# Chthi/Ofighters

Measured on AMD Instinct MI355X. Metric: arena-steps/sec (env.step+obs+policy fwd) at 4096 arenas, 1/2/4/8 MI355X, higher is better.
Workload: dtype f32; 1 GPU; 4096 arenas x 8 ships per GPU, random-bot actions + step + 2D obs rasterise (u8 maps) + bi-head policy forward for 8 ship(s)/arena, trunk shared per arena (BASELINE configs[3]); arenas_per_gpu=4096, ships=8, laser_cap=512, episode_ticks=200, parallelism=arena-sharded x1, RCCL all-reduce of episodic scores only, laser_overflow=0, last_episode_score_sum=70993, last_episode_arenas=4096

## Files before the change

### include/ofx.h

```cpp
#ifndef OFX_H
#define OFX_H

#include <stddef.h>
#include <stdint.h>

#ifdef __cplusplus
extern "C" {
#endif

#define OFX_VERSION 1

enum {
  OFX_OK = 0,
  OFX_ERR_INVALID = -1,
  OFX_ERR_NO_DEVICE = -2,
  OFX_ERR_HIP = -3,
  OFX_ERR_STATE = -4,
  OFX_ERR_OVERFLOW = -5
};

typedef struct ofx_config {
  int32_t n_arenas;
  int32_t n_ships;
  int32_t laser_cap;
// ... 103 lines not shown
int ofx_map_desc(ofx_handle *h, int map_type, int which, ofx_tensor_desc *out);

int ofx_overflow_count(ofx_handle *h, int64_t *count_host);

int ofx_episode_scores(ofx_handle *h, int64_t *sums);
int ofx_episode_scores_grouped(ofx_handle *h, const int32_t *group, int32_t n_groups, int64_t *sums);
int ofx_scores_allreduce(ofx_handle *h, void *nccl_comm, int64_t *sums);

int ofx_scratch_feed(ofx_handle *h, const int32_t *layers_host, int32_t n_layers,
                     const double *weights, const double *biases, const double *x,
                     int32_t batch, double *y, int32_t *argmax);
int ofx_scratch_feed_obs(ofx_handle *h, const int32_t *layers_host, int32_t n_layers,
                         const double *weights, const double *biases, double *y,
                         int32_t *argmax);

typedef struct ofx_policy_desc {
  int32_t n_floats;
  int32_t offset[64];
  int32_t count[64];
  int32_t n_tensors;
} ofx_policy_desc;
int ofx_policy_layout(const ofx_handle *h, ofx_policy_desc *desc_host);
int ofx_policy_forward(ofx_handle *h, const float *weights, const uint8_t *ship_mask,
                       float *act_values, int32_t *iaction, int32_t *ipointer,
                       float *heatmap);
int ofx_policy_pin_weights(ofx_handle *h, const float *weights);
#define OFX_OPT_TRUNK_PLAIN 1
#define OFX_OPT_FRAMES_REF  2
#define OFX_OPT_TRUNK_FUSE  4
#define OFX_OPT_BILINEAR_LEGACY 3
#define OFX_OPT_POLICY_BF16 5
#define OFX_OPT_FIT_PLAIN 6
#define OFX_OPT_TRUNK_SPARSE 7
int ofx_policy_trunk_stats(ofx_handle *h, int64_t *counts_host);
int ofx_set_option(ofx_handle *h, int32_t option, int32_t value);
int ofx_policy_explore(ofx_handle *h, double epsilon, uint64_t seed, uint32_t tick, int32_t collecting,
                       const uint8_t *ship_mask, int32_t *iaction, int32_t *ipointer);
int ofx_policy_epsilon_ladder(ofx_handle *h, const double *expo_host);
int ofx_policy_epsilon_ladder_host(ofx_handle *h, double *dst_host);
int ofx_policy_act(ofx_handle *h, const float *weights, const uint8_t *ship_mask, double epsilon, uint64_t seed,
                   uint32_t tick, int32_t collecting, float *q_sa, float *p_sp, float *v_act, float *v_ptr);
int ofx_policy_actions(ofx_handle *h, const int32_t *iaction, const int32_t *ipointer,
                       const uint8_t *ship_mask, ofx_action *actions);

typedef struct ofx_transition {
  int32_t tick_prev, tick_next;
  int32_t frame_prev, frame_next;
  int32_t ship;
  int32_t iaction, px, py;
  int32_t reward;
  int32_t done;
  float head_prev[8], head_next[8];
} ofx_transition;
int ofx_replay_create(ofx_handle *h, int32_t capacity, int32_t frames);
int ofx_replay_destroy(ofx_handle *h);
int ofx_replay_capture(ofx_handle *h, uint32_t tick, const uint8_t *ship_mask, const int32_t *iaction,
                       const int32_t *ipointer);
int ofx_agents_first_done(ofx_handle *h, const uint8_t *ship_mask, uint8_t *seen, int32_t *count_host);
int ofx_replay_count(ofx_handle *h, int32_t *count_host, int64_t *appended_host);
int ofx_replay_rows_host(ofx_handle *h, int32_t arena, ofx_transition *rows_host, int32_t *n_host);
int ofx_replay_frame_host(ofx_handle *h, int32_t arena, int32_t tick, void *ship_bits_host, void *laser_bits_host);
int ofx_replay_sample(ofx_handle *h, uint64_t seed, uint32_t draw, int32_t batch, int32_t *slot, int32_t *n_sampled);
int ofx_replay_gather(ofx_handle *h, const int32_t *slot, int32_t batch, ofx_transition *rows, void *bits_prev,
                      void *bits_next);
int ofx_replay_gather_valid(ofx_handle *h, const int32_t *slot, const int32_t *n_sampled, int32_t batch, int32_t first,
                            int32_t max_rows, ofx_transition *rows, void *bits_prev, void *bits_next,
// ... 89 lines not shown
```

### ofighters_amd/_native.py

```python
import ctypes as C
import os

_HERE = os.path.dirname(os.path.abspath(__file__))
LIB_PATH = os.path.join(_HERE, "libofx.so")

OFX_OK = 0
OFX_ERR_INVALID = -1
OFX_ERR_NO_DEVICE = -2
OFX_ERR_HIP = -3
OFX_ERR_STATE = -4
OFX_ERR_OVERFLOW = -5

BOT_IDLE, BOT_RANDOM, BOT_TURRET, BOT_RUNNER, BOT_THRUST, BOT_SHOOT = range(6)
BEHAVIOURS = {None: BOT_IDLE, "idle": BOT_IDLE, "random": BOT_RANDOM, "turret": BOT_TURRET,
              "runner": BOT_RUNNER, "thrust": BOT_THRUST, "shoot": BOT_SHOOT}

(F_SHIP_X, F_SHIP_Y, F_SHIP_PX, F_SHIP_PY, F_SHIP_ALIVE, F_REWARD, F_SCORE, F_N_LASERS, F_LASER_X, F_LASER_Y,
 F_LASER_OWNER, F_LASER_DEAD, F_KILLER, F_TIME, F_LAST_SCORES, F_HULL, F_LASER_DX, F_LASER_DY,
 F_OBS_REWARD) = range(19)

MAP_U8, MAP_F32, MAP_F64, MAP_BITS = range(4)
OPT_TRUNK_PLAIN, OPT_FRAMES_REF, OPT_BILINEAR_LEGACY, OPT_TRUNK_FUSE, OPT_POLICY_BF16, OPT_FIT_PLAIN, OPT_TRUNK_SPARSE = 1, 2, 3, 4, 5, 6, 7


class OfxError(Exception):
    def __init__(self, code, msg):
        super().__init__(msg)
        self.code = code


class OfxConfig(C.Structure):
    _fields_ = [(n, C.c_int32) for n in (
        "n_arenas", "n_ships", "laser_cap", "width", "height", "ship_radius", "laser_radius",
        "ship_speed", "laser_speed", "reward_death", "reward_kill", "reward_aim",
        "reward_trajectory", "episode_ticks", "device", "arena_base")]


class OfxAction(C.Structure):
    _fields_ = [("px", C.c_int32), ("py", C.c_int32), ("shoot", C.c_uint8), ("thrust", C.c_uint8),
                ("valid", C.c_uint8), ("_pad", C.c_uint8)]


class OfxTransition(C.Structure):
    _fields_ = [("tick_prev", C.c_int32), ("tick_next", C.c_int32), ("frame_prev", C.c_int32),
                ("frame_next", C.c_int32), ("ship", C.c_int32), ("iaction", C.c_int32),
                ("px", C.c_int32), ("py", C.c_int32), ("reward", C.c_int32), ("done", C.c_int32),
                ("head_prev", C.c_float * 8), ("head_next", C.c_float * 8)]


class OfxTensorDesc(C.Structure):
    _fields_ = [("data", C.c_void_p), ("dtype", C.c_int32), ("itemsize", C.c_int32), ("ndim", C.c_int32),
                ("device", C.c_int32), ("shape", C.c_int64 * 4), ("stride", C.c_int64 * 4)]


DT_U8, DT_I16, DT_I32, DT_I64, DT_F32, DT_F64 = range(6)
# ... 139 lines not shown
```

### ofighters_amd/csrc/ofx_head.hip

```cpp
#include "ofx_head.h"
#include "ofx_lowp.h"
#include "ofx_diag.h"
#include <stdlib.h>


typedef float f32x4 __attribute__((ext_vector_type(4)));
typedef float f32x2 __attribute__((ext_vector_type(2)));
#define HD_PS 400
constexpr int HC4_ZERO = 800;
constexpr int HC4_COL = 816, HC4_CPITCH = 416;
constexpr int HC4_STRIDE = HC4_COL + 2 * HC4_CPITCH + 16;
__device__ __forceinline__ int hc4_at(int ln, int t) { return ln < 2 ? ln * 400 + t : HC4_COL + (ln - 2) * HC4_CPITCH + t; }
__device__ __forceinline__ int hc4_pad(int k) { return k < 16 ? HC4_ZERO + k : k < 32 ? HC4_COL + 400 + k - 16 : HC4_COL + HC4_CPITCH + 400 + k - 32; }

__device__ __forceinline__ void hc4_zero_block(const HeadParams2 &p, int tid, int threads) {
  if (blockIdx.x == 0)
    for (int e = tid; e < HC4_STRIDE; e += threads) p.c4[(size_t)p.S * HC4_STRIDE + e] = 0.f;
}

__device__ __forceinline__ float hd_max_raw(float x, float floor) {
  float pinf;
  asm("s_mov_b32 %0, 0x7f800000" : "=s"(pinf));
  return __builtin_amdgcn_fmed3f(x, floor, pinf);
}

__device__ __forceinline__ unsigned hd_ordered_f32(float v) {
  const unsigned u = __float_as_uint(v);
  return (u & 0x80000000u) ? ~u : (u | 0x80000000u);
}

__global__ __launch_bounds__(1024) void k_head_compact(int S, const uint8_t *mask, int32_t *live) {
  __shared__ int cnt[1024];
  const int t = threadIdx.x, per = (S + 1023) / 1024, lo = min(t * per, S), hi = min(lo + per, S);
  int c = 0;
  for (int s = lo; s < hi; s++) c += mask[s] != 0;
  cnt[t] = c;
  __syncthreads();
  for (int d = 1; d < 1024; d <<= 1) {
    const int v = t >= d ? cnt[t - d] : 0;
    __syncthreads();
    cnt[t] += v;
    __syncthreads();
  }
  int o = cnt[t] - c;
  for (int s = lo; s < hi; s++)
    if (mask[s]) live[1 + o++] = s;
  if (t == 1023) live[0] = cnt[1023];
}

__device__ __forceinline__ int hd_ship(const HeadParams2 &p, int i) {
  if (p.live) return i < p.live[0] ? p.live[1 + i] : -1;
  return i < p.S ? i : -1;
}


__device__ __forceinline__ void hf_taps(int u, int n, int &ka, int &kb, float &w, int legacy) {
  const int k = u >> 1;
  if (legacy) { ka = k; kb = k + 1; w = (u & 1) ? 0.5f : 0.f; }
  else if (u & 1) { ka = k; kb = k + 1; w = 0.25f; } else { ka = k - 1; kb = k; w = 0.75f; }
  ka = min(max(ka, 0), n - 1);
  kb = min(max(kb, 0), n - 1);
}
__device__ __forceinline__ float hf_up(const float *L, int stride, int n, int u, int legacy) {
  int ka, kb; float w;
  hf_taps(u, n, ka, kb, w, legacy);
  const float a = L[ka * stride], b = L[kb * stride];
  return a + (b - a) * w;
}

constexpr int HF_THREADS = 512;
constexpr int HF_L1 = 0;
constexpr int HF_U1R = HF_L1 + 5000;
constexpr int HF_U1C = HF_U1R + 6 * 2 * 102;
constexpr int HF_A_END = HF_U1C + 6 * 2 * 102;
constexpr int HF_U2R = 0;
constexpr int HF_U2C = HF_U2R + 4 * 4 * 202;
static_assert(HF_U2C + 4 * 4 * 202 <= HF_A_END, "region A");
constexpr int HF_B2R = HF_A_END;
constexpr int HF_B2C = HF_B2R + 1600;
constexpr int HF_U3L = HF_B2C + 1600;
constexpr int HF_TOTAL = HF_U3L + 6400;

__global__ __launch_bounds__(HF_THREADS) void k_head_frames_ref(HeadParams2 p) {
  __shared__ __align__(16) float sm[HF_TOTAL];
  const int tid = threadIdx.x;
  const int s = hd_ship(p, (int)blockIdx.x);
  hc4_zero_block(p, tid, HF_THREADS);
  if (s < 0) return;
  float *l1 = sm + HF_L1, *U1r = sm + HF_U1R, *U1c = sm + HF_U1C, *U2r = sm + HF_U2R, *U2c = sm + HF_U2C;
  float *u2rb = sm + HF_B2R, *u2cb = sm + HF_B2C, *u3l = sm + HF_U3L;

  for (int e = tid; e < 5000; e += HF_THREADS) l1[e] = p.up1[(size_t)s * 5000 + e];
  __syncthreads();

  for (int e = tid; e < 2 * 6 * 2 * 102; e += HF_THREADS) {
// ... 101 lines not shown
  __syncthreads();
  for (int e = tid; e < 4 * 200 * 9; e += HF_THREADS) {
    const int tp = e % 9, cell = e / 9;
    float acc = 0.f;
    for (int ci = 0; ci < 8; ci++) acc = fmaf(p.w4raw[tp * 8 + ci], u3l[cell * 8 + ci], acc);
    p.vfr[(size_t)s * 7200 + e] = acc;
  }

  for (int e = tid; e < 4 * 400; e += HF_THREADS) {
    const int ln = e / 400, t = e - ln * 400, isc = ln >> 1, side = ln & 1;
    float acc = 0.f;
    if (!isc || (t > 0 && t < 399)) {
      const int d0 = side ? 2 : 0;
#pragma unroll
      for (int d1 = 0; d1 < 3; d1++)
#pragma unroll
        for (int ci = 0; ci < 8; ci++) {
          const int tap = isc ? d1 * 3 + d0 : d0 * 3 + d1;
          acc += p.w4raw[tap * 8 + ci] * hf_up(u3l + ln * 1600 + ci, 8, 200, t + d1 - 1, p.legacy);
        }
      if (!isc && (t == 0 || t == 399)) {
        const int cl = t ? 3 : 2, dx = t ? 2 : 0;
        for (int dy = 0; dy < 3; dy++) {
          if (dy == d0) continue;
          const int yy = (side ? 399 : 0) + dy - 1;
          if (yy < 0 || yy > 399) continue;
          for (int ci = 0; ci < 8; ci++) acc += p.w4raw[(dy * 3 + dx) * 8 + ci] * hf_up(u3l + cl * 1600 + ci, 8, 200, yy, p.legacy);
        }
      }
    }
    p.c4[(size_t)s * HC4_STRIDE + hc4_at(ln, t)] = acc;
  }
  if (tid < 64) p.c4[(size_t)s * HC4_STRIDE + hc4_pad(tid)] = 0.f;
}

constexpr int HG_THREADS = 256;
constexpr int HG_L1 = 0;
constexpr int HG_U3 = 0;
constexpr int HG_RB = 6400;
constexpr int HG_CB = HG_RB + 4 * 102 * 4;
constexpr int HG_TOTAL = HG_CB + 4 * 102 * 4;
static_assert(2 * 52 * 52 <= 6400, "l1p fits under u3l");

template <int CIN, int COUT, class G>
__device__ __forceinline__ float hg_corner(G get, int n, int yc, int xc, const float *w, float bias, int co, int legacy) {
  float acc = bias;
  for (int dy = 0; dy < 3; dy++) {
    const int uy = yc + dy - 1;
    if (uy < 0 || uy >= 2 * n) continue;
    int ya, yb; float wy;
    hf_taps(uy, n, ya, yb, wy, legacy);
    for (int dx = 0; dx < 3; dx++) {
      const int ux = xc + dx - 1;
      if (ux < 0 || ux >= 2 * n) continue;
      int xa, xb; float wx;
      hf_taps(ux, n, xa, xb, wx, legacy);
      for (int ci = 0; ci < CIN; ci++) {
        const float a = get(ya, xa, ci), b = get(ya, xb, ci), d = get(yb, xa, ci), g = get(yb, xb, ci);
        const float top = a + (b - a) * wx, bot = d + (g - d) * wx;
        acc += w[((dy * 3 + dx) * CIN + ci) * COUT + co] * (top + (bot - top) * wy);
      }
    }
  }
  return fmaxf(acc, 0.f);
}

__global__ __launch_bounds__(HG_THREADS) void k_head_frames(HeadParams2 p) {
  __shared__ __align__(16) float sm[HG_TOTAL];
  __shared__ float efr_s[192], w4s[72];
  const int s = hd_ship(p, (int)((blockIdx.x & ~7u) | ((blockIdx.x + (blockIdx.x >> 3)) & 7u)));
  const int tid = threadIdx.x, lane = tid & 63;
  hc4_zero_block(p, tid, HG_THREADS);
  if (s < 0) return;
  const int wv = __builtin_amdgcn_readfirstlane(tid >> 6);
  const int n16 = lane & 15, kq = lane >> 4;
  float *l1p = sm + HG_L1, *u2rb = sm + HG_RB, *u2cb = sm + HG_CB, *u3l = sm + HG_U3;

  {
    constexpr int NB = 6 * 52 + 46 * 6, NE = 2 * NB, PER = (NE + HG_THREADS - 1) / HG_THREADS;
    float v[PER];
    int at[PER];
#pragma unroll
    for (int u = 0; u < PER; u++) {
      const int e = min(u * HG_THREADS + tid, NE - 1);
      const int ci = e / NB, k = e - ci * NB;
      int r, c;
      if (k < 6 * 52) { const int rr = k / 52; r = rr < 3 ? rr : rr + 46; c = k - rr * 52; }
      else { const int k2 = k - 6 * 52, cc = k2 % 6; r = 3 + k2 / 6; c = cc < 3 ? cc : cc + 46; }
      at[u] = (ci * 52 + r) * 52 + c;
      v[u] = p.up1[(size_t)s * 5000 + (ci * 50 + min(max(r - 1, 0), 49)) * 50 + min(max(c - 1, 0), 49)];
    }
#pragma unroll
    for (int u = 0; u < PER; u++)
      if (u * HG_THREADS + tid < NE) l1p[at[u]] = v[u];
  }
  if (tid < 192) efr_s[tid] = p.efr[tid];
  if (tid < 72) w4s[tid] = p.w4raw[tid];
// ... 668 lines not shown

int ofx_head_compact(ofx_handle *h, int S, const uint8_t *mask, int32_t *live) {
  hipLaunchKernelGGL(k_head_compact, dim3(1), dim3(1024), 0, h->stream, S, mask, live);
  OFX_HIP(hipGetLastError());
  return OFX_OK;
}

size_t ofx_head_frame_bytes(size_t S, size_t *u2fr, size_t *vfr, size_t *c4) {
  *u2fr = 4 * S * 1600;
  *vfr = 4 * S * 7200;
  *c4 = 4 * (S + 1) * HC4_STRIDE;
  return *u2fr + *vfr + *c4;
}

int ofx_launch_head(ofx_handle *h, const HeadParams2 &p0) {
  HeadParams2 p = p0;
#if OFX_HEAD_HOOKS
  { const char *e = getenv("OFX_HEAD_ABLATE"); p.ablate = e ? atoi(e) : 0; }
  static unsigned long long *dbg = nullptr;
  static int dbg_calls = 0;
  const unsigned dbg_blocks = (unsigned)(((p.S + 7) / 8) * 16);
  p.dbg = nullptr;
  if (getenv("OFX_HEAD_STAMPS")) {
    if (!dbg) (void)hipMalloc(&dbg, (size_t)dbg_blocks * 6 * (HS_NB + 4) * 8);
    if (++dbg_calls == 20) p.dbg = dbg;
  }
#endif
  if (p.mask) {
    if (!p.live) { ofx_set_error("ofx_launch_head: a mask needs the live-list scratch"); return OFX_ERR_STATE; }
    if (!p.live_ready) hipLaunchKernelGGL(k_head_compact, dim3(1), dim3(1024), 0, h->stream, p.S, p.mask, p.live);
  } else {
    p.live = nullptr;
  }
  if (p.frames_ref) hipLaunchKernelGGL(k_head_frames_ref, dim3((unsigned)p.S), dim3(HF_THREADS), 0, h->stream, p);
  else hipLaunchKernelGGL(k_head_frames, dim3((unsigned)((p.S + 7) & ~7)), dim3(HG_THREADS), 0, h->stream, p);
  OFX_HIP(hipGetLastError());
  const unsigned blocks = (unsigned)(((p.S + 7) / 8) * 16);
  int rc;
  if (p.event_base >= 0 && (rc = ofx_event_record(h, p.event_base))) return rc;
  const bool extra = p.heat || p.ptr_probe;
#define HS_LAUNCH(E, L) hipLaunchKernelGGL((k_head_stream<E, L>), dim3(blocks), dim3(HS_THREADS), 0, h->stream, p)
  if (p.bf16 == 1) { if (extra) HS_LAUNCH(true, 1); else HS_LAUNCH(false, 1); }
  else if (p.bf16 == 2) { if (extra) HS_LAUNCH(true, 2); else HS_LAUNCH(false, 2); }
  else { if (extra) HS_LAUNCH(true, 0); else HS_LAUNCH(false, 0); }
#undef HS_LAUNCH
  OFX_HIP(hipGetLastError());
  if (p.event_base >= 0 && (rc = ofx_event_record(h, p.event_base + 1))) return rc;
#if OFX_HEAD_HOOKS
  if (p.dbg) {
    (void)hipStreamSynchronize(h->stream);
    unsigned long long *hst = (unsigned long long *)malloc((size_t)blocks * 6 * (HS_NB + 4) * 8);
    (void)hipMemcpy(hst, p.dbg, (size_t)blocks * 6 * (HS_NB + 4) * 8, hipMemcpyDeviceToHost);
    double sum[2][6] = {{0}};
    for (unsigned b = 0; b < blocks; b++)
      for (int w = 0; w < HS_NB + 4; w++)
        for (int i = 0; i < 6; i++) sum[w >= HS_NB][i] += (double)hst[((size_t)b * (HS_NB + 4) + w) * 6 + i] / (w >= HS_NB ? 4.0 : (double)HS_NB);
    for (int r = 0; r < 2; r++) {
      fprintf(stderr, "head stamps %s (cycles per wave and sub-step):", r ? "C" : "B");
      for (int i = 0; i < 6; i++) fprintf(stderr, " %.0f", sum[r][i] / ((double)blocks * HS_NS));
      fprintf(stderr, "\n");
    }
    free(hst);
  }
#endif
  return OFX_OK;
}
```

### ofighters_amd/csrc/ofx_internal.h

```cpp
#pragma once
#include <hip/hip_runtime.h>
#include <stdint.h>
#include <stdio.h>

#include "../../include/ofx.h"

#define OFX_WAVE 64
#define OFX_ARENAS_PER_BLOCK 4

void ofx_set_error(const char *fmt, ...);

#define OFX_HIP(call)                                                                  \
  do {                                                                                 \
    hipError_t _e = (call);                                                            \
    if (_e != hipSuccess) {                                                            \
      ofx_set_error("%s failed: %s (%s:%d)", #call, hipGetErrorString(_e), __FILE__,   \
                    __LINE__);                                                         \
      return OFX_ERR_HIP;                                                              \
    }                                                                                  \
  } while (0)

struct ofx_state {
  int32_t *ship_x, *ship_y, *ship_px, *ship_py, *hull;
  int32_t *reward, *score, *obs_reward, *last_score;
// ... 13 lines not shown
  hipStream_t stream;
  bool own_stream;
  bool spawned;
  ofx_state st;
  double hit_thresh;
  void *maps[5][2];
  int32_t *bot_behaviours;
  void *scratch;
  size_t scratch_bytes;
  hipEvent_t ev0, ev1;
  bool events;
  hipEvent_t *ring;
  int ring_n;
  int prof_base;
  ofx_replay *replay;
  void *aux;
  size_t aux_bytes;
  void *fitws;
  size_t fitws_bytes;
  void *fitws2;
  size_t fitws2_bytes;
  void *applyws;
  size_t applyws_bytes;
  int32_t *counter;
  int32_t *res_iaction;
  int32_t *res_ipointer;
  float *prep;
  float *prep_tmp;
  const float *prep_pinned;
  int opt_trunk_fuse;
  int n_cus;
  bool opt_trunk_plain, opt_frames_ref, opt_bilinear_legacy;
  int opt_policy_lowp;
  bool opt_fit_plain;
  bool opt_trunk_dense, opt_trunk_count;
  unsigned long long *trunk_stat;
  float *act_vals;
  bool act_called;
  double *eps_expo;
};
#define OFX_RING_MAX 65536

int ofx_launch_step(ofx_handle *h, const ofx_action *actions);
int ofx_launch_raster(ofx_handle *h, int map_type, void *ship_map, void *laser_map);
int ofx_ensure_buffer(ofx_handle *h, void **buf, size_t *have, size_t bytes);
int ofx_ensure_scratch(ofx_handle *h, size_t bytes);
enum { OFX_COUNTER_PADS, OFX_COUNTER_FIRST_DONE };
int ofx_counter(ofx_handle *h, int slot, int32_t **counter);
int ofx_policy_results(ofx_handle *h, int32_t **iaction, int32_t **ipointer);
int ofx_policy_act_values(ofx_handle *h, const float **q_sa, const float **p_sp, const float **v_act, const float **v_ptr);
void ofx_replay_free(ofx_handle *h);
int ofx_replay_episode_reset(ofx_handle *h, const uint8_t *arena_mask);
int ofx_launch_gemm(ofx_handle *h, const float *A, int lda, const float *B, int ldb, const float *bias, float *C, int ldc,
                    int M, int N, int K, int relu, const int32_t *live = nullptr);
int ofx_policy_weights_updated(ofx_handle *h, const float *weights);
int ofx_policy_predict_obs(ofx_handle *h, const float *weights, int32_t n_obs, const void *bits, const float *vec8,
                           float *act_values, float *heatmap, float *ptr_max);

#define OFX_MAP_BITS_LSB 4

__host__ __device__ inline void ofx_philox4x32_10(uint32_t c0, uint32_t c1, uint32_t c2, uint32_t c3,
                                                  uint32_t k0, uint32_t k1, uint32_t out[4]) {
#pragma unroll
  for (int r = 0; r < 10; r++) {
    uint64_t p0 = (uint64_t)0xD2511F53u * c0, p1 = (uint64_t)0xCD9E8D57u * c2;
    uint32_t n0 = (uint32_t)(p1 >> 32) ^ c1 ^ k0, n1 = (uint32_t)p1;
// ... 14 lines not shown
```

### ofighters_amd/csrc/ofx_policy.hip

```cpp
#include <string.h>

#include "ofx_internal.h"
#include "ofx_blob.h"
#include "ofx_trunk.h"
#include "ofx_head.h"

typedef float f32x16 __attribute__((ext_vector_type(16)));


extern "C" int ofx_policy_layout(const ofx_handle *h, ofx_policy_desc *desc) {
  (void)h;
  if (!desc) { ofx_set_error("ofx_policy_layout: null desc"); return OFX_ERR_INVALID; }
  memset(desc, 0, sizeof(*desc));
  desc->n_tensors = policy_layout(desc->offset, desc->count);
  desc->n_floats = desc->offset[desc->n_tensors];
  return OFX_OK;
}

struct PrepLayout {
  int tw[4], tb[4];
  int uw[3], ub[3];
  int w3mf;
  int w2mf;
  int w2fr;
  int w3fr;
  int w4eff_c;
  int w4raw;
  int efr;
  int b4;
  int zero16;
  int wbm[3];
  int lut1;
  int total;
};

static PrepLayout prep_layout() {
  PrepLayout L;
  int off = 0;
// ... 440 lines not shown
  pp.legacy = h->opt_bilinear_legacy;
  pp.phase = 0;
  hipLaunchKernelGGL(k_policy_prepare, dim3(32), dim3(256), 0, h->stream, pp);
  pp.phase = 1;
  hipLaunchKernelGGL(k_policy_prepare, dim3(4), dim3(256), 0, h->stream, pp);
  OFX_HIP(hipGetLastError());
  return OFX_OK;
}

extern "C" int ofx_policy_pin_weights(ofx_handle *h, const float *weights) {
  if (!h) { ofx_set_error("ofx_policy_pin_weights: null handle"); return OFX_ERR_INVALID; }
  OFX_HIP(hipSetDevice(h->cfg.device));
  h->prep_pinned = nullptr;
  if (!weights) return OFX_OK;
  int rc = policy_prepare(h, weights, &h->prep);
  if (rc) return rc;
  h->prep_pinned = weights;
  return OFX_OK;
}

int ofx_policy_weights_updated(ofx_handle *h, const float *weights) {
  if (h->prep_pinned && h->prep_pinned == weights) return policy_prepare(h, weights, &h->prep);
  return OFX_OK;
}

extern "C" int ofx_set_option(ofx_handle *h, int32_t option, int32_t value) {
  if (!h) { ofx_set_error("ofx_set_option: null handle"); return OFX_ERR_INVALID; }
  switch (option) {
    case OFX_OPT_TRUNK_PLAIN: h->opt_trunk_plain = value != 0; return OFX_OK;
    case OFX_OPT_TRUNK_FUSE:
      if (value < 0 || value > 2) { ofx_set_error("ofx_set_option: OFX_OPT_TRUNK_FUSE takes 0 (auto), 1 (always), 2 (never)"); return OFX_ERR_INVALID; }
      h->opt_trunk_fuse = value; return OFX_OK;
    case OFX_OPT_FRAMES_REF: h->opt_frames_ref = value != 0; return OFX_OK;
    case OFX_OPT_TRUNK_SPARSE:
      if (value && !h->trunk_stat) {
        OFX_HIP(hipSetDevice(h->cfg.device));
        OFX_HIP(hipMalloc((void **)&h->trunk_stat, 4 * sizeof(unsigned long long)));
        OFX_HIP(hipMemsetAsync(h->trunk_stat, 0, 4 * sizeof(unsigned long long), h->stream));
      }
      h->opt_trunk_dense = value == 0; h->opt_trunk_count = value != 0; return OFX_OK;
    case OFX_OPT_FIT_PLAIN: h->opt_fit_plain = value != 0; return OFX_OK;
    case OFX_OPT_POLICY_BF16:
      if (value < 0 || value > 2) { ofx_set_error("ofx_set_option: OFX_OPT_POLICY_BF16 takes 0 (fp32), 1 (bf16 operands), 2 (fp16 operands)"); return OFX_ERR_INVALID; }
      h->opt_policy_lowp = value; return OFX_OK;
    case OFX_OPT_BILINEAR_LEGACY:
      if (h->opt_bilinear_legacy == (value != 0)) return OFX_OK;
      h->opt_bilinear_legacy = value != 0;
      OFX_HIP(hipSetDevice(h->cfg.device));
      return h->prep_pinned ? policy_prepare(h, h->prep_pinned, &h->prep) : OFX_OK;
    default: ofx_set_error("ofx_set_option: unknown option %d", option); return OFX_ERR_INVALID;
  }
}

struct ForwardArgs {
  const float *weights;
  int N, M;
  const unsigned *bits[2];
  size_t bits_stride;
  const float *vec8;
  const uint8_t *ship_mask;
  float *act_values, *heatmap, *ptr_max, *ptr_probe;
  int32_t *iaction, *ipointer;
  const int32_t *probe;
};

static int policy_forward_impl(ofx_handle *h, const ForwardArgs &a) {
// ... 15 lines not shown
  memset(&tp, 0, sizeof(tp));
  tp.bits[0] = a.bits[0]; tp.bits[1] = a.bits[1]; tp.bits_stride = a.bits_stride; tp.images = N;
  for (int i = 0; i < 4; i++) { tp.tw[i] = prep + L.tw[i]; tp.tb[i] = prep + L.tb[i]; }
  for (int i = 0; i < 3; i++) tp.wbm[i] = prep + L.wbm[i];
  tp.lut1 = prep + L.lut1; tp.zero16 = prep + L.zero16;
  tp.p1 = ws.p1; tp.p2 = ws.p2; tp.p3 = ws.p3; tp.p4 = ws.p4;
  tp.lowp = lowp; tp.sparse = !h->opt_trunk_dense || a.vec8 != nullptr;
  tp.stat = h->opt_trunk_count ? h->trunk_stat : nullptr;
  if ((rc = ofx_launch_trunk(h, tp))) return rc;

  const float *k1 = weights + off[OFX_T_DENSE1];
  {
    const int tiles = ((N + 31) / 32) * 4, jobs = tiles * kDense1Chunks;
    hipLaunchKernelGGL(k_gemm_f32_splitk, dim3((jobs + 3) / 4), dim3(256), 0, h->stream, ws.p4, 5000, k1 + 8 * 100, 100,
                       ws.g1, N, 100, 5000 / kDense1Chunks, tiles, jobs);
    OFX_HIP(hipGetLastError());
  }
  HeadParams hp;
  hp.N = N; hp.M = a.M; hp.st = h->st; hp.vec8 = a.vec8; hp.g1 = ws.g1; hp.g1_chunks = kDense1Chunks;
  hp.k1 = k1; hp.b1 = weights + off[OFX_T_DENSE1 + 1];
  hp.k2 = weights + off[OFX_T_DENSE2]; hp.b2 = weights + off[OFX_T_DENSE2 + 1];
  hp.k3 = weights + off[OFX_T_OUT1]; hp.b3 = weights + off[OFX_T_OUT1 + 1];
  const int32_t *live = nullptr;
  if (a.ship_mask) {
    if ((rc = ofx_head_compact(h, S, a.ship_mask, ws.live))) return rc;
    live = ws.live;
  }
  hp.mask = a.ship_mask; hp.live = live; hp.d1 = ws.d1; hp.act = a.act_values; hp.iaction = a.iaction ? a.iaction : ws.iaction;
  hipLaunchKernelGGL(k_head_dense, dim3((S + 3) / 4), dim3(256), 0, h->stream, hp);
  OFX_HIP(hipGetLastError());

  if ((rc = ofx_launch_gemm(h, ws.d1, 100, weights + off[OFX_T_UPDENSE], 625, weights + off[OFX_T_UPDENSE + 1], ws.u0, 625, S, 625, 100, 1, live)))
    return rc;
  ConvParams up;
  memset(&up, 0, sizeof(up));
  up.live = live; up.images = S; up.legacy = h->opt_bilinear_legacy;
  up.in = ws.u0; up.w = prep + L.uw[0]; up.b = prep + L.ub[0]; up.out = ws.up1;
  hipLaunchKernelGGL(k_upconv1, dim3((unsigned)(live && S > 4096 ? 4096 : S)), dim3(256), 0, h->stream, up);
  OFX_HIP(hipGetLastError());
  OFX_HIP(hipMemsetAsync(ws.best, 0, sizeof(unsigned long long) * S, h->stream));
  HeadParams2 hp2;
  memset(&hp2, 0, sizeof(hp2));
  hp2.S = S; hp2.up1 = ws.up1;
  hp2.w2mf = prep + L.w2mf; hp2.b2 = prep + L.ub[1]; hp2.w2raw = prep + L.uw[1];
  hp2.w3mf = prep + L.w3mf; hp2.b3 = prep + L.ub[2]; hp2.w3raw = prep + L.uw[2];
  hp2.w4eff_c = prep + L.w4eff_c; hp2.b4 = prep + L.b4; hp2.w4raw = prep + L.w4raw;
  hp2.w2fr = prep + L.w2fr; hp2.w3fr = prep + L.w3fr; hp2.efr = prep + L.efr;
  hp2.u2fr = ws.u2fr; hp2.vfr = ws.vfr; hp2.c4 = ws.c4;
  hp2.frames_ref = h->opt_frames_ref; hp2.legacy = h->opt_bilinear_legacy;
  hp2.bf16 = lowp;
  hp2.mask = a.ship_mask; hp2.live = ws.live; hp2.live_ready = a.ship_mask != nullptr; hp2.best = ws.best; hp2.heat = a.heatmap;
  hp2.probe = a.probe; hp2.ptr_probe = a.probe ? a.ptr_probe : nullptr;
  const int pb = h->prof_base;
  hp2.event_base = pb;
  if ((rc = ofx_launch_head(h, hp2))) return rc;
  if (pb >= 0) h->prof_base = pb + 3 < OFX_RING_MAX ? pb + 2 : -1;
  hipLaunchKernelGGL(k_policy_finish, dim3((S + 255) / 256), dim3(256), 0, h->stream, S, a.ship_mask, ws.best,
                     a.ipointer ? a.ipointer : ws.ipointer, a.ptr_max);
  OFX_HIP(hipGetLastError());
  return OFX_OK;
}

static int live_forward_check(ofx_handle *h, const float *weights, const char *who) {
  if (!h || !weights) { ofx_set_error("%s: null argument", who); return OFX_ERR_INVALID; }
  if (!h->spawned) { ofx_set_error("You must execute analyse_battleground first."); return OFX_ERR_STATE; }
  const ofx_config &c = h->cfg;
  if (c.width != PS || c.height != PS) {
    ofx_set_error("%s: the pointer_model takes 400x400 maps (got %d x %d)", who, c.width, c.height);
    return OFX_ERR_INVALID;
  }
  return OFX_OK;
}

static int live_forward(ofx_handle *h, ForwardArgs &a) {
  const ofx_config &c = h->cfg;
  int rc = ofx_launch_raster(h, OFX_MAP_BITS_LSB, nullptr, nullptr);
  if (rc) return rc;
  int32_t *ria, *rip;
  if ((rc = ofx_policy_results(h, &ria, &rip))) return rc;
  if (!a.iaction) a.iaction = ria;
  if (!a.ipointer) a.ipointer = rip;
  a.N = c.n_arenas; a.M = c.n_ships;
  a.bits[0] = (const unsigned *)h->maps[OFX_MAP_BITS_LSB][0]; a.bits[1] = (const unsigned *)h->maps[OFX_MAP_BITS_LSB][1];
  a.bits_stride = (size_t)(PS * PS) >> 5;
  return policy_forward_impl(h, a);
// ... 223 lines not shown
```

Measured before the change: 228,900 arena-steps/s.

## Fuse first upconv into head frames kernel as default front path

Adds a k_head_front kernel that performs the first bilinear upsample and 3x3 conv from the 25x25 dense output in shared memory, then continues straight into the frame/edge computations that k_head_frames did. The fused kernel is the default, so k_upconv1 is no longer launched. The l1 plane stays on chip instead of being re-read from global memory, which removes one kernel launch and a round trip of intermediate activations. up1 is still written out for later stages, and the fused kernel's larger register and LDS footprint may lower occupancy.

```diff
diff --git a/include/ofx.h b/include/ofx.h
--- a/include/ofx.h
+++ b/include/ofx.h
@@ -159,6 +159,7 @@
 #define OFX_OPT_POLICY_BF16 5
 #define OFX_OPT_FIT_PLAIN 6
 #define OFX_OPT_TRUNK_SPARSE 7
+#define OFX_OPT_HEAD_FRONT 8
 int ofx_policy_trunk_stats(ofx_handle *h, int64_t *counts_host);
 int ofx_set_option(ofx_handle *h, int32_t option, int32_t value);
 int ofx_policy_explore(ofx_handle *h, double epsilon, uint64_t seed, uint32_t tick, int32_t collecting,
diff --git a/ofighters_amd/_native.py b/ofighters_amd/_native.py
--- a/ofighters_amd/_native.py
+++ b/ofighters_amd/_native.py
@@ -20,7 +20,7 @@
  F_OBS_REWARD) = range(19)
 
 MAP_U8, MAP_F32, MAP_F64, MAP_BITS = range(4)
-OPT_TRUNK_PLAIN, OPT_FRAMES_REF, OPT_BILINEAR_LEGACY, OPT_TRUNK_FUSE, OPT_POLICY_BF16, OPT_FIT_PLAIN, OPT_TRUNK_SPARSE = 1, 2, 3, 4, 5, 6, 7
+OPT_TRUNK_PLAIN, OPT_FRAMES_REF, OPT_BILINEAR_LEGACY, OPT_TRUNK_FUSE, OPT_POLICY_BF16, OPT_FIT_PLAIN, OPT_TRUNK_SPARSE, OPT_HEAD_FRONT = 1, 2, 3, 4, 5, 6, 7, 8
 
 
 class OfxError(Exception):
diff --git a/ofighters_amd/csrc/ofx_front.h b/ofighters_amd/csrc/ofx_front.h
--- /dev/null
+++ b/ofighters_amd/csrc/ofx_front.h
@@ -0,0 +1,11 @@
+#pragma once
+#include "ofx_head.h"
+
+struct FrontParams {
+  HeadParams2 h;
+  const float *u0;
+  const float *w1, *b1;
+  float *up1;
+};
+
+int ofx_launch_front(ofx_handle *h, const FrontParams &p);
diff --git a/ofighters_amd/csrc/ofx_front.hip b/ofighters_amd/csrc/ofx_front.hip
--- /dev/null
+++ b/ofighters_amd/csrc/ofx_front.hip
@@ -0,0 +1,325 @@
+#include "ofx_front.h"
+#include "ofx_head_frames.h"
+
+template <int M0, int CNT>
+__device__ __forceinline__ void hfr_line_tiles(const float *band, int v, int n16, int kq, const float (&bw3)[9], float bias, float *u3l) {
+  const int b0 = (v & 1) ? 2 : 0;
+  f32x4 d[CNT];
+  int qq[CNT];
+#pragma unroll
+  for (int mm = 0; mm < CNT; mm++) {
+    d[mm] = (f32x4){bias, bias, bias, bias};
+    qq[mm] = min(16 * (M0 + mm) + n16, 99);
+  }
+#pragma unroll
+  for (int jj = 0; jj < 9; jj++) {
+    const int ty = jj / 3, tx = jj % 3;
+    const int tf = v < 2 ? ty : tx, ta = v < 2 ? tx : ty;
+    const int bsel = (v & 1) ? b0 + min(tf, 1) : b0 + max(tf - 1, 0);
+#pragma unroll
+    for (int mm = 0; mm < CNT; mm++) {
+      const float a = band[(bsel * 102 + qq[mm] + ta) * 4 + kq];
+      d[mm] = __builtin_amdgcn_mfma_f32_16x16x4f32(a, bw3[jj], d[mm], 0, 0, 0);
+    }
+  }
+  const int co = n16 & 7, par = n16 >> 3;
+#pragma unroll
+  for (int mm = 0; mm < CNT; mm++)
+#pragma unroll
+    for (int r = 0; r < 4; r++) {
+      const int q = 16 * (M0 + mm) + 4 * kq + r;
+      if (q < 100) u3l[(v * 200 + 2 * q + par) * 8 + co] = fmaxf(d[mm][r], 0.f);
+    }
+}
+
+typedef float f32x2 __attribute__((ext_vector_type(2)));
+template <class T>
+__device__ __forceinline__ void hfr_store(T *dst, T v) { __builtin_nontemporal_store(v, dst); }
+
+constexpr int HFR_UP = HG_RB, HFR_UPP = 53;
+static_assert(52 * HFR_UPP <= HG_TOTAL - HG_RB, "the up-sampled plane fits where the bands stand later");
+
+__global__ __launch_bounds__(HG_THREADS) void k_head_front(FrontParams fp) {
+  const HeadParams2 &p = fp.h;
+  __shared__ __align__(16) float sm[HG_TOTAL];
+  __shared__ float efr_s[192], w4s[72], w3s[288], b3s[8];
+  static_assert(4 * (HG_TOTAL + 192 + 72 + 288 + 8) <= 160 * 1024 / 4, "four workgroups per CU");
+  const int s = hd_ship(p, (int)((blockIdx.x & ~7u) | ((blockIdx.x + (blockIdx.x >> 3)) & 7u)));
+  const int tid = threadIdx.x, lane = tid & 63;
+  hc4_zero_block(p, tid, HG_THREADS);
+  if (s < 0) return;
+  const int wv = __builtin_amdgcn_readfirstlane(tid >> 6);
+  const int n16 = lane & 15, kq = lane >> 4;
+  float *u0s = sm, *up = sm + HFR_UP;
+  float *l1p = sm + HG_L1, *u2rb = sm + HG_RB, *u2cb = sm + HG_CB, *u3l = sm + HG_U3;
+  float *w2s = sm + 2 * 52 * 52, *b2s = w2s + 72, *w1s = b2s + 4, *b1s = w1s + 18;
+  static_assert(2 * 52 * 52 + 72 + 4 + 18 + 2 <= HG_RB, "w2raw, b2, w1 and b1 fit behind l1p");
+
+  const float *u0g = fp.u0 + (size_t)s * 625;
+  const float g0 = u0g[tid], g1 = u0g[tid + 256], g2 = u0g[min(tid + 512, 624)];
+  const float ge = p.efr[min(tid, 191)], g4 = p.w4raw[min(tid, 71)], gw2 = p.w2raw[min(tid, 71)], gb2 = p.b2[tid & 3];
+  const float gw3 = p.w3raw[tid], gw3b = p.w3raw[256 + (tid & 31)], gb3 = p.b3[tid & 7];
+  const float gw1 = fp.w1[min(tid, 17)], gb1 = fp.b1[tid & 1];
+  const float bias2 = p.b2[n16 & 3], bias3 = p.b3[n16 & 7];
+  float bw2[5];
+#pragma unroll
+  for (int jj = 0; jj < 5; jj++) bw2[jj] = p.w2fr[(wv * 20 + 4 * jj + kq) * 16 + n16];
+  float bw3[9];
+#pragma unroll
+  for (int jj = 0; jj < 9; jj++) bw3[jj] = p.w3fr[(wv * 36 + 4 * jj + kq) * 16 + n16];
+  u0s[tid] = g0; u0s[tid + 256] = g1;
+  if (tid + 512 < 625) u0s[tid + 512] = g2;
+  if (tid < 192) efr_s[tid] = ge;
+  if (tid < 72) { w4s[tid] = g4; w2s[tid] = gw2; }
+  if (tid < 4) b2s[tid] = gb2;
+  if (tid < 18) w1s[tid] = gw1;
+  if (tid < 2) b1s[tid] = gb1;
+  w3s[tid] = gw3;
+  if (tid < 32) w3s[256 + tid] = gw3b;
+  if (tid < 8) b3s[tid] = gb3;
+  __syncthreads();
+  if (tid < 4 * 52) {
+    const int c = tid % 52, rg = tid / 52, gx = c - 1;
+    const bool inx = gx >= 0 && gx < 50;
+    const float sx = p.legacy ? (float)gx * 0.5f : ((float)gx + 0.5f) * 0.5f - 0.5f;
+    const float fx = floorf(sx), lx = sx - fx;
+    const int x0 = min(max((int)fx, 0), 24), x1 = min(max((int)fx + 1, 0), 24);
+#pragma unroll
+    for (int k = 0; k < 13; k++) {
+      const int r = rg + 4 * k, gy = r - 1;
+      const float sy = p.legacy ? (float)gy * 0.5f : ((float)gy + 0.5f) * 0.5f - 0.5f;
+      const float fy = floorf(sy), ly = sy - fy;
+      const int y0 = min(max((int)fy, 0), 24), y1 = min(max((int)fy + 1, 0), 24);
+      const float a = u0s[y0 * 25 + x0], b = u0s[y0 * 25 + x1], d = u0s[y1 * 25 + x0], g = u0s[y1 * 25 + x1];
+      const float top = __builtin_fmaf(b - a, lx, a), bot = __builtin_fmaf(g - d, lx, d);
+      const float v = __builtin_fmaf(bot - top, ly, top);
+      up[r * HFR_UPP + c] = (inx && gy >= 0 && gy < 50) ? v : 0.f;
+    }
+  }
+  __syncthreads();
+
+  if (tid < 250) {
+    const int row = tid / 5, seg = tid - 5 * row, x0 = 10 * seg;
+    float acc[2][10];
+#pragma unroll
+    for (int co = 0; co < 2; co++)
+#pragma unroll
+      for (int i = 0; i < 10; i++) acc[co][i] = 0.f;
+#pragma unroll
+    for (int dy = 0; dy < 3; dy++) {
+      float v[12];
+#pragma unroll
+      for (int i = 0; i < 12; i++) v[i] = up[(row + dy) * HFR_UPP + x0 + i];
+#pragma unroll
+      for (int dx = 0; dx < 3; dx++)
+#pragma unroll
+        for (int co = 0; co < 2; co++) {
+          const float wgt = w1s[(dy * 3 + dx) * 2 + co];
+#pragma unroll
+          for (int i = 0; i < 10; i++) acc[co][i] = __builtin_fmaf(v[i + dx], wgt, acc[co][i]);
+        }
+    }
+    const bool frow = row < 2 || row >= 48;
+    const int r1 = row + 1, r2 = row == 0 ? 0 : row == 49 ? 51 : -1;
+#pragma unroll
+    for (int co = 0; co < 2; co++) {
+      const float bias = b1s[co];
+#pragma unroll
+      for (int i = 0; i < 10; i++) acc[co][i] = fmaxf(acc[co][i] + bias, 0.f);
+      float *o = fp.up1 + (((size_t)s * 2 + co) * 50 + row) * 50 + x0;
+      const float *a = acc[co];
+      if (((row + seg) & 1) == 0) {
+        hfr_store(reinterpret_cast<f32x4 *>(o), (f32x4){a[0], a[1], a[2], a[3]});
+        hfr_store(reinterpret_cast<f32x4 *>(o + 4), (f32x4){a[4], a[5], a[6], a[7]});
+        hfr_store(reinterpret_cast<f32x2 *>(o + 8), (f32x2){a[8], a[9]});
+      } else {
+        hfr_store(reinterpret_cast<f32x2 *>(o), (f32x2){a[0], a[1]});
+        hfr_store(reinterpret_cast<f32x4 *>(o + 2), (f32x4){a[2], a[3], a[4], a[5]});
+        hfr_store(reinterpret_cast<f32x4 *>(o + 6), (f32x4){a[6], a[7], a[8], a[9]});
+      }
+      float *pl = l1p + co * 52 * 52;
+#pragma unroll
+      for (int i = 0; i < 10; i++) {
+        const int x = x0 + i;
+        if (frow || x < 2 || x >= 48) {
+          const int c1 = x + 1, c2 = x == 0 ? 0 : x == 49 ? 51 : -1;
+          pl[r1 * 52 + c1] = a[i];
+          if (r2 >= 0) pl[r2 * 52 + c1] = a[i];
+          if (c2 >= 0) {
+            pl[r1 * 52 + c2] = a[i];
+            if (r2 >= 0) pl[r2 * 52 + c2] = a[i];
+          }
+        }
+      }
+    }
+  }
+  __syncthreads();
+
+  {
+    const int v = wv;
+    const float bias = bias2;
+    f32x4 d[4];
+    int i[4], j[4];
+#pragma unroll
+    for (int m = 0; m < 4; m++) {
+      const int pp = min(16 * m + n16, 49);
+      i[m] = v == 0 ? 0 : v == 1 ? 49 : pp; j[m] = v == 2 ? 0 : v == 3 ? 49 : pp;
+      d[m] = (f32x4){bias, bias, bias, bias};
+    }
+#pragma unroll
+    for (int jj = 0; jj < 5; jj++) {
+      const int tap = min(2 * jj + (kq >> 1), 8);
+#pragma unroll
+      for (int m = 0; m < 4; m++) {
+        const float a = l1p[((kq & 1) * 52 + i[m] + tap / 3) * 52 + j[m] + tap % 3];
+        d[m] = __builtin_amdgcn_mfma_f32_16x16x4f32(a, bw2[jj], d[m], 0, 0, 0);
+      }
+    }
+    const int co = n16 & 3, pa = n16 >> 3, pb = (n16 >> 2) & 1;
+#pragma unroll
+    for (int m = 0; m < 4; m++)
+#pragma unroll
+      for (int r = 0; r < 4; r++) {
+        const int q = 16 * m + 4 * kq + r;
+        if (q >= 50) continue;
+        const float val = fmaxf(d[m][r], 0.f);
+        if (v < 2) {
+          u2rb[((2 * v + pa) * 102 + 2 * q + pb + 1) * 4 + co] = val;
+        } else {
+          u2cb[((2 * (v - 2) + pb) * 102 + 2 * q + pa + 1) * 4 + co] = val;
+        }
+      }
+  }
+  __syncthreads();
+  if (tid < 64) {
+    const int co = tid & 3, cx = (tid >> 2) & 1, cy = (tid >> 3) & 1, bx = (tid >> 4) & 1, by = tid >> 5;
+    const int y = by ? 98 + cy : cy, x = bx ? 98 + cx : cx;
+    const int rb = by ? 2 + cy : cy, cb = bx ? 2 + cx : cx;
+    const bool fy = y == 0 || y == 99, fx = x == 0 || x == 99;
+    float val;
+    if (fy && fx) {
+      auto get = [&](int yy, int xx, int ci) { return l1p[(ci * 52 + yy + 1) * 52 + xx + 1]; };
+      val = hg_corner<2, 4>(get, 50, y, x, w2s, b2s[co], co, p.legacy);
+    } else if (fx) {
+      val = u2cb[(cb * 102 + y + 1) * 4 + co];
+    } else {
+      val = u2rb[(rb * 102 + x + 1) * 4 + co];
+    }
+    if (fy && fx) { u2rb[(rb * 102 + x + 1) * 4 + co] = val; u2cb[(cb * 102 + y + 1) * 4 + co] = val; }
+    else if (fx) u2rb[(rb * 102 + x + 1) * 4 + co] = val;
+    else u2cb[(cb * 102 + y + 1) * 4 + co] = val;
+  }
+  __syncthreads();
+  if (tid < 128) {
+    const int co = tid & 3, b = (tid >> 2) & 3, hi = (tid >> 4) & 1, isc = tid >> 5;
+    if (isc < 2) {
+      float *ln = (isc ? u2cb : u2rb) + b * 102 * 4;
+      ln[(hi ? 101 : 0) * 4 + co] = ln[(hi ? 100 : 1) * 4 + co];
+    }
+  }
+  for (int e = tid; e < 4 * 100; e += HG_THREADS) {
+    const int ln = e / 100, r = e - ln * 100;
+    const float *src = ln < 2 ? u2rb + (ln ? 3 : 0) * 408 : u2cb + (ln == 3 ? 3 : 0) * 408;
+    hfr_store(reinterpret_cast<f32x4 *>(p.u2fr + (size_t)s * 1600 + 4 * e), *reinterpret_cast<const f32x4 *>(src + 4 + 4 * r));
+  }
+  __syncthreads();
+
+  {
+    const float *band = wv < 2 ? u2rb : u2cb;
+    const float bias = bias3;
+    hfr_line_tiles<0, 4>(band, wv, n16, kq, bw3, bias, u3l);
+    hfr_line_tiles<4, 3>(band, wv, n16, kq, bw3, bias, u3l);
+  }
+  __syncthreads();
+  if (tid < 32) {
+    const int co = tid & 7, c = tid >> 3;
+    const int y = (c & 1) ? 199 : 0, x = (c & 2) ? 199 : 0;
+    auto get = [&](int yy, int xx, int ci) {
+      return u2rb[((yy < 50 ? yy : yy - 96) * 102 + xx + 1) * 4 + ci];
+    };
+    const float val = hg_corner<4, 8>(get, 100, y, x, w3s, b3s[co], co, p.legacy);
+    u3l[(((c & 1) ? 1 : 0) * 200 + x) * 8 + co] = val;
+    u3l[(((c & 2) ? 3 : 2) * 200 + y) * 8 + co] = val;
+  }
+  __syncthreads();
+
+  if (tid < 252) {
+    float wt[4][8];
+    int cof[4];
+#pragma unroll
+    for (int i = 0; i < 4; i++) {
+      const int e = 4 * tid + i, tp = e % 9;
+      cof[i] = (e / 9) * 8;
+#pragma unroll
+      for (int ci = 0; ci < 8; ci++) wt[i][ci] = w4s[tp * 8 + ci];
+    }
+    float *dst = p.vfr + (size_t)s * 7200 + 4 * tid;
+#pragma unroll 2
+    for (int k = 0; k < 8; k++) {
+      if (tid + 252 * k >= 1800) break;
+      f32x4 out;
+#pragma unroll
+      for (int i = 0; i < 4; i++) {
+        const float *cell = u3l + cof[i] + 112 * 8 * k;
+        const f32x4 ua = *reinterpret_cast<const f32x4 *>(cell), ub = *reinterpret_cast<const f32x4 *>(cell + 4);
+        float acc = 0.f;
+#pragma unroll
+        for (int ci = 0; ci < 4; ci++) acc = __builtin_fmaf(wt[i][ci], ua[ci], acc);
+#pragma unroll
+        for (int ci = 0; ci < 4; ci++) acc = __builtin_fmaf(wt[i][4 + ci], ub[ci], acc);
+        out[i] = acc;
+      }
+      hfr_store(reinterpret_cast<f32x4 *>(dst + 1008 * k), out);
+    }
+  }
+
+  {
+    const int ln = wv, isc = ln >> 1, side = ln & 1, b = lane & 1;
+    float E[24];
+#pragma unroll
+    for (int k = 0; k < 24; k++) E[k] = efr_s[(ln * 2 + b) * 24 + k];
+    const float *L = u3l + ln * 1600;
+    for (int t = lane; t < 400; t += 64) {
+      const int jq = t >> 1;
+      float acc = 0.f;
+      if (!isc || (t > 0 && t < 399)) {
+#pragma unroll
+        for (int o = 0; o < 3; o++) {
+          const float *Lp = L + min(max(jq + o - 1, 0), 199) * 8;
+          const f32x4 ua = *reinterpret_cast<const f32x4 *>(Lp), ub = *reinterpret_cast<const f32x4 *>(Lp + 4);
+#pragma unroll
+          for (int ci = 0; ci < 4; ci++) acc = __builtin_fmaf(E[o * 8 + ci], ua[ci], acc);
+#pragma unroll
+          for (int ci = 0; ci < 4; ci++) acc = __builtin_fmaf(E[o * 8 + 4 + ci], ub[ci], acc);
+        }
+        if (!isc && (t == 0 || t == 399)) {
+          const int cs = t ? 1 : 0;
+          const int yq = side ? 199 : 0, a = side ? 1 : 0;
+          const float *E2 = efr_s + ((2 + cs) * 2 + a) * 24;
+          const float *L2 = u3l + (2 + cs) * 1600;
+          for (int o = 0; o < 3; o++) {
+            const float *Lp = L2 + min(max(yq + o - 1, 0), 199) * 8;
+            for (int ci = 0; ci < 8; ci++) acc = __builtin_fmaf(E2[o * 8 + ci], Lp[ci], acc);
+          }
+          const int tap = (side ? 2 : 0) * 3 + (cs ? 2 : 0);
+          const float *Lc = L + (t ? 199 : 0) * 8;
+          for (int ci = 0; ci < 8; ci++) acc = __builtin_fmaf(-w4s[tap * 8 + ci], Lc[ci], acc);
+        }
+      }
+      hfr_store(p.c4 + (size_t)s * HC4_STRIDE + hc4_at(ln, t), acc);
+    }
+  }
+  if (tid < 64) p.c4[(size_t)s * HC4_STRIDE + hc4_pad(tid)] = 0.f;
+}
+
+int ofx_launch_front(ofx_handle *h, const FrontParams &p0) {
+  FrontParams p = p0;
+  if (p.h.mask) {
+    if (!p.h.live || !p.h.live_ready) { ofx_set_error("ofx_launch_front: a mask needs the ordered list of its ships"); return OFX_ERR_STATE; }
+  } else {
+    p.h.live = nullptr;
+  }
+  hipLaunchKernelGGL(k_head_front, dim3((unsigned)((p.h.S + 7) & ~7)), dim3(HG_THREADS), 0, h->stream, p);
+  OFX_HIP(hipGetLastError());
+  return OFX_OK;
+}
diff --git a/ofighters_amd/csrc/ofx_head.hip b/ofighters_amd/csrc/ofx_head.hip
--- a/ofighters_amd/csrc/ofx_head.hip
+++ b/ofighters_amd/csrc/ofx_head.hip
@@ -1,23 +1,12 @@
 #include "ofx_head.h"
+#include "ofx_head_frames.h"
 #include "ofx_lowp.h"
 #include "ofx_diag.h"
 #include <stdlib.h>
 
 
-typedef float f32x4 __attribute__((ext_vector_type(4)));
 typedef float f32x2 __attribute__((ext_vector_type(2)));
 #define HD_PS 400
-constexpr int HC4_ZERO = 800;
-constexpr int HC4_COL = 816, HC4_CPITCH = 416;
-constexpr int HC4_STRIDE = HC4_COL + 2 * HC4_CPITCH + 16;
-__device__ __forceinline__ int hc4_at(int ln, int t) { return ln < 2 ? ln * 400 + t : HC4_COL + (ln - 2) * HC4_CPITCH + t; }
-__device__ __forceinline__ int hc4_pad(int k) { return k < 16 ? HC4_ZERO + k : k < 32 ? HC4_COL + 400 + k - 16 : HC4_COL + HC4_CPITCH + 400 + k - 32; }
-
-__device__ __forceinline__ void hc4_zero_block(const HeadParams2 &p, int tid, int threads) {
-  if (blockIdx.x == 0)
-    for (int e = tid; e < HC4_STRIDE; e += threads) p.c4[(size_t)p.S * HC4_STRIDE + e] = 0.f;
-}
-
 __device__ __forceinline__ float hd_max_raw(float x, float floor) {
   float pinf;
   asm("s_mov_b32 %0, 0x7f800000" : "=s"(pinf));
@@ -48,19 +37,7 @@
   if (t == 1023) live[0] = cnt[1023];
 }
 
-__device__ __forceinline__ int hd_ship(const HeadParams2 &p, int i) {
-  if (p.live) return i < p.live[0] ? p.live[1 + i] : -1;
-  return i < p.S ? i : -1;
-}
-
-
-__device__ __forceinline__ void hf_taps(int u, int n, int &ka, int &kb, float &w, int legacy) {
-  const int k = u >> 1;
-  if (legacy) { ka = k; kb = k + 1; w = (u & 1) ? 0.5f : 0.f; }
-  else if (u & 1) { ka = k; kb = k + 1; w = 0.25f; } else { ka = k - 1; kb = k; w = 0.75f; }
-  ka = min(max(ka, 0), n - 1);
-  kb = min(max(kb, 0), n - 1);
-}
+
 __device__ __forceinline__ float hf_up(const float *L, int stride, int n, int u, int legacy) {
   int ka, kb; float w;
   hf_taps(u, n, ka, kb, w, legacy);
@@ -228,37 +205,6 @@
     p.c4[(size_t)s * HC4_STRIDE + hc4_at(ln, t)] = acc;
   }
   if (tid < 64) p.c4[(size_t)s * HC4_STRIDE + hc4_pad(tid)] = 0.f;
-}
-
-constexpr int HG_THREADS = 256;
-constexpr int HG_L1 = 0;
-constexpr int HG_U3 = 0;
-constexpr int HG_RB = 6400;
-constexpr int HG_CB = HG_RB + 4 * 102 * 4;
-constexpr int HG_TOTAL = HG_CB + 4 * 102 * 4;
-static_assert(2 * 52 * 52 <= 6400, "l1p fits under u3l");
-
-template <int CIN, int COUT, class G>
-__device__ __forceinline__ float hg_corner(G get, int n, int yc, int xc, const float *w, float bias, int co, int legacy) {
-  float acc = bias;
-  for (int dy = 0; dy < 3; dy++) {
-    const int uy = yc + dy - 1;
-    if (uy < 0 || uy >= 2 * n) continue;
-    int ya, yb; float wy;
-    hf_taps(uy, n, ya, yb, wy, legacy);
-    for (int dx = 0; dx < 3; dx++) {
-      const int ux = xc + dx - 1;
-      if (ux < 0 || ux >= 2 * n) continue;
-      int xa, xb; float wx;
-      hf_taps(ux, n, xa, xb, wx, legacy);
-      for (int ci = 0; ci < CIN; ci++) {
-        const float a = get(ya, xa, ci), b = get(ya, xb, ci), d = get(yb, xa, ci), g = get(yb, xb, ci);
-        const float top = a + (b - a) * wx, bot = d + (g - d) * wx;
-        acc += w[((dy * 3 + dx) * CIN + ci) * COUT + co] * (top + (bot - top) * wy);
-      }
-    }
-  }
-  return fmaxf(acc, 0.f);
 }
 
 __global__ __launch_bounds__(HG_THREADS) void k_head_frames(HeadParams2 p) {
@@ -993,7 +939,8 @@
   } else {
     p.live = nullptr;
   }
-  if (p.frames_ref) hipLaunchKernelGGL(k_head_frames_ref, dim3((unsigned)p.S), dim3(HF_THREADS), 0, h->stream, p);
+  if (p.frames_ref == 2) { }
+  else if (p.frames_ref) hipLaunchKernelGGL(k_head_frames_ref, dim3((unsigned)p.S), dim3(HF_THREADS), 0, h->stream, p);
   else hipLaunchKernelGGL(k_head_frames, dim3((unsigned)((p.S + 7) & ~7)), dim3(HG_THREADS), 0, h->stream, p);
   OFX_HIP(hipGetLastError());
   const unsigned blocks = (unsigned)(((p.S + 7) / 8) * 16);
diff --git a/ofighters_amd/csrc/ofx_head_frames.h b/ofighters_amd/csrc/ofx_head_frames.h
--- /dev/null
+++ b/ofighters_amd/csrc/ofx_head_frames.h
@@ -0,0 +1,59 @@
+#pragma once
+#include "ofx_head.h"
+
+typedef float f32x4 __attribute__((ext_vector_type(4)));
+
+constexpr int HC4_ZERO = 800;
+constexpr int HC4_COL = 816, HC4_CPITCH = 416;
+constexpr int HC4_STRIDE = HC4_COL + 2 * HC4_CPITCH + 16;
+__device__ __forceinline__ int hc4_at(int ln, int t) { return ln < 2 ? ln * 400 + t : HC4_COL + (ln - 2) * HC4_CPITCH + t; }
+__device__ __forceinline__ int hc4_pad(int k) { return k < 16 ? HC4_ZERO + k : k < 32 ? HC4_COL + 400 + k - 16 : HC4_COL + HC4_CPITCH + 400 + k - 32; }
+
+__device__ __forceinline__ void hc4_zero_block(const HeadParams2 &p, int tid, int threads) {
+  if (blockIdx.x == 0)
+    for (int e = tid; e < HC4_STRIDE; e += threads) p.c4[(size_t)p.S * HC4_STRIDE + e] = 0.f;
+}
+
+__device__ __forceinline__ int hd_ship(const HeadParams2 &p, int i) {
+  if (p.live) return i < p.live[0] ? p.live[1 + i] : -1;
+  return i < p.S ? i : -1;
+}
+
+__device__ __forceinline__ void hf_taps(int u, int n, int &ka, int &kb, float &w, int legacy) {
+  const int k = u >> 1;
+  if (legacy) { ka = k; kb = k + 1; w = (u & 1) ? 0.5f : 0.f; }
+  else if (u & 1) { ka = k; kb = k + 1; w = 0.25f; } else { ka = k - 1; kb = k; w = 0.75f; }
+  ka = min(max(ka, 0), n - 1);
+  kb = min(max(kb, 0), n - 1);
+}
+
+constexpr int HG_THREADS = 256;
+constexpr int HG_L1 = 0;
+constexpr int HG_U3 = 0;
+constexpr int HG_RB = 6400;
+constexpr int HG_CB = HG_RB + 4 * 102 * 4;
+constexpr int HG_TOTAL = HG_CB + 4 * 102 * 4;
+static_assert(2 * 52 * 52 <= 6400, "l1p fits under u3l");
+
+template <int CIN, int COUT, class G>
+__device__ __forceinline__ float hg_corner(G get, int n, int yc, int xc, const float *w, float bias, int co, int legacy) {
+  float acc = bias;
+  for (int dy = 0; dy < 3; dy++) {
+    const int uy = yc + dy - 1;
+    if (uy < 0 || uy >= 2 * n) continue;
+    int ya, yb; float wy;
+    hf_taps(uy, n, ya, yb, wy, legacy);
+    for (int dx = 0; dx < 3; dx++) {
+      const int ux = xc + dx - 1;
+      if (ux < 0 || ux >= 2 * n) continue;
+      int xa, xb; float wx;
+      hf_taps(ux, n, xa, xb, wx, legacy);
+      for (int ci = 0; ci < CIN; ci++) {
+        const float a = get(ya, xa, ci), b = get(ya, xb, ci), d = get(yb, xa, ci), g = get(yb, xb, ci);
+        const float top = a + (b - a) * wx, bot = d + (g - d) * wx;
+        acc += w[((dy * 3 + dx) * CIN + ci) * COUT + co] * (top + (bot - top) * wy);
+      }
+    }
+  }
+  return fmaxf(acc, 0.f);
+}
diff --git a/ofighters_amd/csrc/ofx_internal.h b/ofighters_amd/csrc/ofx_internal.h
--- a/ofighters_amd/csrc/ofx_internal.h
+++ b/ofighters_amd/csrc/ofx_internal.h
@@ -69,6 +69,7 @@
   int n_cus;
   bool opt_trunk_plain, opt_frames_ref, opt_bilinear_legacy;
   int opt_policy_lowp;
+  bool opt_front_split;
   bool opt_fit_plain;
   bool opt_trunk_dense, opt_trunk_count;
   unsigned long long *trunk_stat;
diff --git a/ofighters_amd/csrc/ofx_policy.hip b/ofighters_amd/csrc/ofx_policy.hip
--- a/ofighters_amd/csrc/ofx_policy.hip
+++ b/ofighters_amd/csrc/ofx_policy.hip
@@ -4,6 +4,7 @@
 #include "ofx_blob.h"
 #include "ofx_trunk.h"
 #include "ofx_head.h"
+#include "ofx_front.h"
 
 typedef float f32x16 __attribute__((ext_vector_type(16)));
 
@@ -510,6 +511,9 @@
       if (value < 0 || value > 2) { ofx_set_error("ofx_set_option: OFX_OPT_TRUNK_FUSE takes 0 (auto), 1 (always), 2 (never)"); return OFX_ERR_INVALID; }
       h->opt_trunk_fuse = value; return OFX_OK;
     case OFX_OPT_FRAMES_REF: h->opt_frames_ref = value != 0; return OFX_OK;
+    case OFX_OPT_HEAD_FRONT:
+      if (value < 0 || value > 1) { ofx_set_error("ofx_set_option: OFX_OPT_HEAD_FRONT takes 1 (one kernel, the default) or 0 (k_upconv1 + k_head_frames)"); return OFX_ERR_INVALID; }
+      h->opt_front_split = value == 0; return OFX_OK;
     case OFX_OPT_TRUNK_SPARSE:
       if (value && !h->trunk_stat) {
         OFX_HIP(hipSetDevice(h->cfg.device));
@@ -591,12 +595,15 @@
 
   if ((rc = ofx_launch_gemm(h, ws.d1, 100, weights + off[OFX_T_UPDENSE], 625, weights + off[OFX_T_UPDENSE + 1], ws.u0, 625, S, 625, 100, 1, live)))
     return rc;
-  ConvParams up;
-  memset(&up, 0, sizeof(up));
-  up.live = live; up.images = S; up.legacy = h->opt_bilinear_legacy;
-  up.in = ws.u0; up.w = prep + L.uw[0]; up.b = prep + L.ub[0]; up.out = ws.up1;
-  hipLaunchKernelGGL(k_upconv1, dim3((unsigned)(live && S > 4096 ? 4096 : S)), dim3(256), 0, h->stream, up);
-  OFX_HIP(hipGetLastError());
+  const bool front = !h->opt_front_split && !h->opt_frames_ref;
+  if (!front) {
+    ConvParams up;
+    memset(&up, 0, sizeof(up));
+    up.live = live; up.images = S; up.legacy = h->opt_bilinear_legacy;
+    up.in = ws.u0; up.w = prep + L.uw[0]; up.b = prep + L.ub[0]; up.out = ws.up1;
+    hipLaunchKernelGGL(k_upconv1, dim3((unsigned)(live && S > 4096 ? 4096 : S)), dim3(256), 0, h->stream, up);
+    OFX_HIP(hipGetLastError());
+  }
   OFX_HIP(hipMemsetAsync(ws.best, 0, sizeof(unsigned long long) * S, h->stream));
   HeadParams2 hp2;
   memset(&hp2, 0, sizeof(hp2));
@@ -606,10 +613,15 @@
   hp2.w4eff_c = prep + L.w4eff_c; hp2.b4 = prep + L.b4; hp2.w4raw = prep + L.w4raw;
   hp2.w2fr = prep + L.w2fr; hp2.w3fr = prep + L.w3fr; hp2.efr = prep + L.efr;
   hp2.u2fr = ws.u2fr; hp2.vfr = ws.vfr; hp2.c4 = ws.c4;
-  hp2.frames_ref = h->opt_frames_ref; hp2.legacy = h->opt_bilinear_legacy;
+  hp2.frames_ref = front ? 2 : h->opt_frames_ref; hp2.legacy = h->opt_bilinear_legacy;
   hp2.bf16 = lowp;
   hp2.mask = a.ship_mask; hp2.live = ws.live; hp2.live_ready = a.ship_mask != nullptr; hp2.best = ws.best; hp2.heat = a.heatmap;
   hp2.probe = a.probe; hp2.ptr_probe = a.probe ? a.ptr_probe : nullptr;
+  if (front) {
+    FrontParams fp;
+    fp.h = hp2; fp.u0 = ws.u0; fp.w1 = prep + L.uw[0]; fp.b1 = prep + L.ub[0]; fp.up1 = ws.up1;
+    if ((rc = ofx_launch_front(h, fp))) return rc;
+  }
   const int pb = h->prof_base;
   hp2.event_base = pb;
   if ((rc = ofx_launch_head(h, hp2))) return rc;
```

Result: no change. 230,800 arena-steps/s (median of 6 runs) (+0.8%).
